# yglbgyx/DS-GAN

Hardware: AMD Instinct MI355X
Metric: 256×256 paired imgs/sec (G+D step) at 1/2/4/8 MI355X; MS-SSIM Δ vs ref (higher is better)
Workload: dtype bf16; 1 GPU; DS-GAN optimize_parameters, MixConvNeXtML G + PatchGAN D + VGG16 perceptual + SSIM/L1/TV; global_batch=16, per_gpu_batch=16, parallelism=dp1, hip_graphs=True

## Files before the change

ds-gan_amd/csrc/mlp.hip:

```cpp
#include "common.h"
#include "lds_dma.h"
#include <type_traits>

namespace dsg {

typedef f32x16_t mf32x16;
typedef __attribute__((ext_vector_type(4))) short ms16x4;
typedef __attribute__((address_space(3))) ms16x4 lds_ms16x4;
typedef __attribute__((ext_vector_type(4))) unsigned int mu32x4;

template <typename T16>
__device__ __forceinline__ hx8<T16> mtr_frag(const T16* p0, int stride) {
#if defined(__HIP_DEVICE_COMPILE__)
  ms16x4 lo = __builtin_amdgcn_ds_read_tr16_b64_v4i16((lds_ms16x4*)(p0));
  ms16x4 hi = __builtin_amdgcn_ds_read_tr16_b64_v4i16((lds_ms16x4*)(p0 + 4 * stride));
  typedef __attribute__((ext_vector_type(8))) short s16x8;
  s16x8 v = {lo[0], lo[1], lo[2], lo[3], hi[0], hi[1], hi[2], hi[3]};
  return __builtin_bit_cast(hx8<T16>, v);
#else
  return hx8<T16>{};
#endif
}

template <typename T16>
// ... 8 lines not shown
template <bool PK>
__device__ __forceinline__ void mlp_gelu_pair2(f32x2 z, f32x2& g, f32x2& gp) {
  if (PK) gelu_pair_fast2(z, g, gp);
  else gelu_pair_fast1x2(z, g, gp);
}
template <bool PK>
__device__ __forceinline__ f32x2 mlp_mul2(f32x2 a, f32x2 b) { return PK ? a * b : f32x2{a.x * b.x, a.y * b.y}; }

struct MlpArgs {
  const void* h; long h_bs;
  const float* dy; long dy_bs;
  const void* w1;
  const float* b1;
  const void* w2;
  const float* b2;
  float* out; long out_bs;
  void* g_out;
  void* dz_out;
  float* bsum;
  int HW, nb, accumulate;
  int h_bf16;
  float* ws;
  int splits;
  const float* x; long x_bs;
  const void* wsc;
};

__device__ __forceinline__ int xcd_tile(int id, int nwg) {
  const int xcd = id & 7, q = nwg >> 3, r = nwg & 7;
  return (xcd < r ? xcd * (q + 1) : r * (q + 1) + (xcd - r) * q) + (id >> 3);
}

template <int K, int BN, int STR, int NT, typename T16>
__device__ __forceinline__ void stage_rows(T16* dst, const float* __restrict__ src, int HW, int tid) {
  constexpr int ITEMS = K * BN / 4;
  static_assert(ITEMS % NT == 0, "tile must split evenly over the workgroup");
  constexpr int PER = ITEMS / NT;
  constexpr int BATCH = PER < 8 ? PER : 8;
#pragma unroll
  for (int i0 = 0; i0 < PER; i0 += BATCH) {
    float4 v[BATCH];
#pragma unroll
    for (int i = 0; i < BATCH; ++i) {
      const int it = tid + (i0 + i) * NT;
      const int k = it / (BN / 4), c4 = it % (BN / 4);
      v[i] = *reinterpret_cast<const float4*>(src + (long)k * HW + c4 * 4);
    }
// ... 450 lines not shown
  return __builtin_bit_cast(hx8<T16>, v);
#else
  return hx8<T16>{};
#endif
}
template <int S, typename T16>
__device__ __forceinline__ hx8<T16> mtr_frag_s(const T16* T, int k0, int col0, int lane) {
#if defined(__HIP_DEVICE_COMPILE__)
  const int tq = (lane >> 2) & 3, tp = lane & 3, tG = (lane >> 4) & 1, h = lane >> 5;
  const int col = col0 + 16 * tG + 4 * tp;
  const int rlo = k0 + 8 * h + tq, rhi = rlo + 4;
  const T16* plo = T + rlo * (S * 8) + (((col >> 3) ^ slot_swz<S>(rlo)) << 3) + (col & 7);
  const T16* phi = T + rhi * (S * 8) + (((col >> 3) ^ slot_swz<S>(rhi)) << 3) + (col & 7);
  ms16x4 lo = __builtin_amdgcn_ds_read_tr16_b64_v4i16((lds_ms16x4*)(plo));
  ms16x4 hi = __builtin_amdgcn_ds_read_tr16_b64_v4i16((lds_ms16x4*)(phi));
  typedef __attribute__((ext_vector_type(8))) short s16x8;
  s16x8 v = {lo[0], lo[1], lo[2], lo[3], hi[0], hi[1], hi[2], hi[3]};
  return __builtin_bit_cast(hx8<T16>, v);
#else
  return hx8<T16>{};
#endif
}

template <typename T16, int C, int P, int MINB>
__global__ __launch_bounds__(512, MINB) void mlp_dh_kernel(MlpArgs g) {
  typedef hx8<T16> mbf16x8;
  typedef hx4<T16> mbf16x4;
  constexpr int NW = 8, NT = NW * 64, BN = 128, HC = 64;
  constexpr int C4 = 4 * C, NCH = C4 / HC, KS = C / 16, PS = P / 16, CT = C / 32;
  constexpr int HSTR = BN + 32;
  constexpr int ST_SZ = (C + P) * HSTR, W_SZ = HC * C + P * HC, R_SZ = 2 * 4 * CT * 16 * 64;
  constexpr int SM = ST_SZ > 2 * W_SZ ? (ST_SZ > R_SZ ? ST_SZ : R_SZ) : (2 * W_SZ > R_SZ ? 2 * W_SZ : R_SZ);
  __shared__ __attribute__((aligned(16))) T16 smem[SM + 2 * C4];
  float* b1s = reinterpret_cast<float*>(smem + SM);
  static_assert(C % 64 == 0 && P % 64 == 0 && NCH >= 2, "tile shape");

  const int tid = threadIdx.x, lane = tid & 63, wave = __builtin_amdgcn_readfirstlane(tid >> 6);
  const int lr = lane & 31, lh = lane >> 5;
  const int tq = (lane >> 2) & 3, tp = lane & 3, tG = (lane >> 4) & 1;
  const int wm = wave >> 2, wn = wave & 3;

  const int tpi = g.HW / BN;
  const int tile = xcd_tile(blockIdx.x, gridDim.x);
  const int img = tile / tpi, p0 = (tile - img * tpi) * BN;

  T16* Hs = smem;
  T16* Ds = smem + C * HSTR;
// ... 64 lines not shown
    raw_barrier();
    if (j + 2 < NCH) {
      T16* W1n = smem + (j & 1) * W_SZ;
      glds_chunk<C, P, NW, false>(W1n, W1n + HC * C, g.w1, g.w2, j + 2, wave, lane);
    }
  }

  float* red = reinterpret_cast<float*>(smem);
#pragma unroll
  for (int ct = 0; ct < CT; ++ct)
    if ((ct & 1) != wm)
#pragma unroll
      for (int r = 0; r < 16; ++r) red[((wn * CT + ct) * 16 + r) * 64 + lane] = hacc[ct][r];
  __syncthreads();
  float* ob = g.out + (long)img * g.out_bs + p0 + wn * 32 + lr;
#pragma unroll
  for (int ct = 0; ct < CT; ++ct)
    if ((ct & 1) == wm)
#pragma unroll
      for (int r = 0; r < 16; ++r) {
        const float o = red[((wn * CT + ct) * 16 + r) * 64 + lane];
        ob[(long)(ct * 32 + (r & 3) + 8 * (r >> 2) + 4 * lh) * g.HW] = wm == 0 ? hacc[ct][r] + o : o + hacc[ct][r];
      }
}

template <typename T16, int C, int P, int BN, int HC, int NW, bool GD, int MINB, bool DMA = false>
__global__ __launch_bounds__(NW * 64, MINB) void mlp_bwd_kernel(MlpArgs g) {
  typedef hx8<T16> mbf16x8;
  typedef hx4<T16> mbf16x4;
  constexpr int NT = NW * 64;
  constexpr int C4 = 4 * C, NCH = C4 / HC;
  constexpr int HSTR = BN + 32, NSTR = HC, W1STR = C, W2STR = HC;
  constexpr int H_SZ = C * HSTR, D_SZ = P * HSTR, N_SZ = BN * NSTR, W1_SZ = HC * W1STR, W2_SZ = P * W2STR;
  constexpr int W_SZ = W1_SZ + W2_SZ;
  static_assert(!DMA || (H_SZ + D_SZ >= W_SZ && HC == 64 && (C / 8) % NW == 0 && (P / 8) % NW == 0), "DMA ring");
  constexpr int SM_SZ = DMA ? H_SZ + D_SZ + W_SZ + (GD ? 2 : 1) * N_SZ + 2 * C4
                            : H_SZ + D_SZ + (GD ? 2 : 1) * N_SZ + W1_SZ + W2_SZ;
  __shared__ __attribute__((aligned(16))) T16 smem[SM_SZ];
  T16* Hs = smem;
  T16* Ds = Hs + H_SZ;
  T16* Zn = Ds + D_SZ + (DMA ? W_SZ : 0);
  T16* Gn = Zn + (GD ? N_SZ : 0);
  T16* W1s = DMA ? Ds + D_SZ : Zn + (GD ? 2 : 1) * N_SZ;
  T16* W2s = W1s + W1_SZ;
  float* b1s = reinterpret_cast<float*>(Zn + (GD ? 2 : 1) * N_SZ);

  using ZG = WGrid<HC, BN, NW>;
  using HG = WGrid<C, BN, NW>;
  static_assert(P % 16 == 0 && HC == 64 && BN % 16 == 0, "tile shape");
// ... 142 lines not shown
          hacc[i][t] = mfma16(af[i], bf[t], hacc[i][t]);
    }
    if constexpr (!DMA) {
      __syncthreads();
      if (j + 1 < NCH) {
        wch_store_swz<C, P, HC, NT>(wr1, wr2, W1s, W2s, tid);
        __syncthreads();
      }
    }
  }

  float* ob = g.out + (long)img * g.out_bs + p0;
#pragma unroll
  for (int i = 0; i < HG::TM; ++i)
#pragma unroll
    for (int t = 0; t < HG::TN; ++t) {
      const int n = wn * (BN / HG::WN) + t * 32 + lr;
#pragma unroll
      for (int r = 0; r < 16; ++r) {
        const int c = wm * (C / 2) + i * 32 + (r & 3) + 8 * (r >> 2) + 4 * lh;
        ob[(long)c * g.HW + n] = hacc[i][t][r];
      }
    }
}

template <int S>
__device__ __forceinline__ unsigned swz_row_b(int row, int lh) {
  return (unsigned)(row * S * 16 + ((lh ^ slot_swz<S>(row)) << 4));
}
template <int S>
__device__ __forceinline__ uint2 swz_tr_b(int col0, int lane) {
  const int tq = (lane >> 2) & 3, tp = lane & 3, tG = (lane >> 4) & 1, h = lane >> 5;
  const int col = col0 + 16 * tG + 4 * tp;
  const int rlo = 8 * h + tq, rhi = rlo + 4;
  return make_uint2((unsigned)(rlo * S * 8 + (((col >> 3) ^ slot_swz<S>(rlo)) << 3) + (col & 7)) * 2u,
                    (unsigned)(rhi * S * 8 + (((col >> 3) ^ slot_swz<S>(rhi)) << 3) + (col & 7)) * 2u);
}
template <typename T16>
__device__ __forceinline__ hx8<T16> tr_at(const T16* T, uint2 a, unsigned k_bytes) {
#if defined(__HIP_DEVICE_COMPILE__)
  const char* b = (const char*)T + k_bytes;
  ms16x4 lo = __builtin_amdgcn_ds_read_tr16_b64_v4i16((lds_ms16x4*)(b + a.x));
  ms16x4 hi = __builtin_amdgcn_ds_read_tr16_b64_v4i16((lds_ms16x4*)(b + a.y));
  typedef __attribute__((ext_vector_type(8))) short s16x8;
  s16x8 v = {lo[0], lo[1], lo[2], lo[3], hi[0], hi[1], hi[2], hi[3]};
  return __builtin_bit_cast(hx8<T16>, v);
#else
  return hx8<T16>{};
#endif
}

template <typename T16, int C, int P>
__global__ __launch_bounds__(256, 1) void mlp_bwd_dma_kernel(MlpArgs g) {
  typedef hx8<T16> mbf16x8;
  typedef hx4<T16> mbf16x4;
  constexpr int NW = 4, NT = 256, BN = 64, HC = 64;
  constexpr int C4 = 4 * C, NCH = C4 / HC;
  constexpr int HSTR = BN + 32;
  constexpr int H_SZ = C * HSTR, D_SZ = P * HSTR, N_SZ = BN * HC, W1_SZ = HC * C, W2_SZ = P * HC;
  constexpr int W_SZ = W1_SZ + W2_SZ;
  static_assert(H_SZ + D_SZ >= W_SZ && NCH % 2 == 0 && (C / 8) % NW == 0 && (P / 8) % NW == 0, "shape");
  __shared__ __attribute__((aligned(1024))) T16 smem[H_SZ + D_SZ + W_SZ + 2 * N_SZ + 2 * C4];
  T16* const Hs = smem;
  T16* const Ds = Hs + H_SZ;
  T16* const Wslot0 = Ds + D_SZ;
  T16* const Wslot1 = Hs;
  T16* const Zn = Wslot0 + W_SZ;
  T16* const Gn = Zn + N_SZ;
  float* const b1s = reinterpret_cast<float*>(Gn + N_SZ);

  const int tid = threadIdx.x, lane = tid & 63, wave = __builtin_amdgcn_readfirstlane(tid >> 6);
  const int lr = lane & 31, lh = lane >> 5;
  const int tq = (lane >> 2) & 3, tp = lane & 3, tG = (lane >> 4) & 1;
  const int wm = wave >> 1, wn = wave & 1;

// ... 118 lines not shown
      dzb[ks] = *reinterpret_cast<const mbf16x8*>((const char*)Zn + (a_n ^ (unsigned)(32 * ks)));
#pragma unroll
      for (int i = 0; i < 4; ++i) w1t[ks][i] = tr_at(W1s, a_d[i], ks * 16 * C * 2);
    }
    __builtin_amdgcn_sched_barrier(0);
#pragma unroll
    for (int ks = 0; ks < HC / 16; ++ks)
#pragma unroll
      for (int i = 0; i < 4; ++i) hacc[i] = mfma16(w1t[ks][i], dzb[ks], hacc[i]);
  };
  for (int j = 0; j < NCH; j += 2) {
    chunk(j, Wslot0, Wslot1);
    chunk(j + 1, Wslot1, Wslot0);
  }

  float* ob = g.out + (long)img * g.out_bs + p0 + wn * 32 + lr;
#pragma unroll
  for (int i = 0; i < 4; ++i)
#pragma unroll
    for (int r = 0; r < 16; ++r) {
      const int c = wm * (C / 2) + i * 32 + (r & 3) + 8 * (r >> 2) + 4 * lh;
      ob[(long)c * g.HW] = hacc[i][r];
    }
}

template <int K, int BN, int NT, bool BF>
struct TileLd {
  static constexpr int E = BF ? 8 : 4;
  static constexpr int N = K * BN / E / NT;
  static_assert((K * BN / E) % NT == 0, "tile split");
  mu32x4 v[N];
  __device__ __forceinline__ void load(const void* src, int HW, int tid) {
#pragma unroll
    for (int i = 0; i < N; ++i) {
      const int it = tid + i * NT, k = it / (BN / E), c = it % (BN / E);
      const char* p = (const char*)src + ((long)k * HW + c * E) * (BF ? 2 : 4);
      v[i] = *reinterpret_cast<const mu32x4*>(p);
    }
  }
  template <int STR, typename T16>
  __device__ __forceinline__ void store(T16* dst, int tid) const {
#pragma unroll
    for (int i = 0; i < N; ++i) {
      const int it = tid + i * NT, k = it / (BN / E), c = it % (BN / E);
      if constexpr (BF) *reinterpret_cast<mu32x4*>(dst + k * STR + c * E) = v[i];
      else *reinterpret_cast<hx4<T16>*>(dst + k * STR + c * E) = mcvt4<T16>(__builtin_bit_cast(float4, v[i]));
// ... 268 lines not shown
static int mlp_bn(int C, int P) {
  if ((C == 64 && P == 128) || (C == 128 && P == 64) || (C == 128 && P == 256) || (C == 256 && P == 128)) return 128;
  return 0;
}
constexpr int MLP_NW = 8;

template <typename T16, int C, int P, int BN, int MINB>
static void fwd_lds_launch(const MlpArgs& g, hipStream_t st) {
  const unsigned tiles = (unsigned)((long)g.nb * (g.HW / BN));
  if (g.x)
    hipLaunchKernelGGL((mlp_fwd_lds_kernel<T16, C, P, BN, 64, MLP_NW, MINB, true>), dim3(tiles), dim3(MLP_NW * 64), 0, st,
                       g);
  else
    hipLaunchKernelGGL((mlp_fwd_lds_kernel<T16, C, P, BN, 64, MLP_NW, MINB>), dim3(tiles), dim3(MLP_NW * 64), 0, st, g);
}
template <typename T16, int C, int P, int MINB>
static void fwd_launch(const MlpArgs& g, hipStream_t st) {
  const unsigned tiles = (unsigned)((long)g.nb * (g.HW / 128));
  if (g.x) hipLaunchKernelGGL((mlp_fwd_kernel<T16, C, P, MINB, true>), dim3(tiles), dim3(512), 0, st, g);
  else hipLaunchKernelGGL((mlp_fwd_kernel<T16, C, P, MINB>), dim3(tiles), dim3(512), 0, st, g);
}
static int g_mlp_tune[4] = {2, 0, 0, 0};

template <typename T16, int C, int P, int BN, int NW, bool GD = true, int MINB = 1, bool DMA = false>
static void bwd_launch(const MlpArgs& g, hipStream_t st) {
  static_assert(BN / (NW / 2) == 32, "bsum granularity");
  const unsigned tiles = (unsigned)((long)g.nb * (g.HW / BN));
  hipLaunchKernelGGL((mlp_bwd_kernel<T16, C, P, BN, 64, NW, GD, MINB, DMA>), dim3(tiles), dim3(NW * 64), 0, st, g);
}

static int mlp_wgrad_splits(int C, int P, int HW, int nb) {
  const int bn = 64;
  const int nch = 4 * C / 64;
  const long ntiles = (long)nb * (HW / bn);
  long S = 512 / nch;
  S = S / 8 * 8;
  if (S < 8) S = 8;
  if (S > ntiles) S = ntiles;
  return (int)S;
}

template <typename T16, int C, int P, int BN, int NW, int MINB>
static void wgrad_launch(const MlpArgs& g, hipStream_t st) {
  const unsigned wgs = (unsigned)((4 * C / 64) * g.splits);
  if (g.h_bf16) hipLaunchKernelGGL((mlp_wgrad_kernel<T16, C, P, BN, NW, true, MINB>), dim3(wgs), dim3(NW * 64), 0, st, g);
  else hipLaunchKernelGGL((mlp_wgrad_kernel<T16, C, P, BN, NW, false, MINB>), dim3(wgs), dim3(NW * 64), 0, st, g);
}

}

using namespace dsg;
// ... 23 lines not shown
    using T16 = std::remove_pointer_t<decltype(t)>;
    if (C == 64) fwd_lds_launch<T16, 64, 128, 128, 2>(g, st);
    else if (C == 128 && P == 64) fwd_launch<T16, 128, 64, 4>(g, st);
    else if (C == 128) fwd_launch<T16, 128, 256, 2>(g, st);
    else fwd_launch<T16, 256, 128, 2>(g, st);
  });
  DSG_CHECK_LAUNCH();
  return 0;
}

int dsgan_mlp_fwd(const void* h, long h_bs, int h_bf16, const void* w1, const float* b1, const void* w2,
                  const float* b2, float* out, long out_bs, int nb, int C, int P, int HW,
                  int accumulate, hipStream_t st) {
  return mlp_fwd_impl(h, h_bs, h_bf16, w1, b1, w2, b2, nullptr, 0, nullptr, out, out_bs, nb, C, P, HW, accumulate, st);
}

int dsgan_mlp_fwd_sc(const void* h, long h_bs, int h_bf16, const void* w1, const float* b1, const void* w2,
                     const float* b2, const float* x, long x_bs, const void* ws, float* out, long out_bs, int nb,
                     int C, int P, int HW, int accumulate, hipStream_t st) {
  DSG_REQUIRE(x && ws, "dsgan_mlp_fwd_sc: bad args");
  return mlp_fwd_impl(h, h_bs, h_bf16, w1, b1, w2, b2, x, x_bs, ws, out, out_bs, nb, C, P, HW, accumulate, st);
}

int dsgan_mlp_bwd(const void* h, long h_bs, int h_bf16, const float* dy, long dy_bs, const void* w1, const float* b1,
                  const void* w2, float* dh, long dh_bs, void* g_out, void* dz_out, float* bsum, int nb,
                  int C, int P, int HW, hipStream_t st) {
  DSG_REQUIRE(h && dy && w1 && b1 && w2 && dh && nb > 0 && (g_out != nullptr) == (dz_out != nullptr) && (g_out || !bsum),
              "dsgan_mlp_bwd: bad args (g_out and dz_out both or neither; bsum needs them)");
  DSG_REQUIRE(dsgan_mlp_supported(C, P, HW), "dsgan_mlp_bwd: unsupported shape C=%d P=%d HW=%d", C, P, HW);
  DSG_REQUIRE(((uintptr_t)h & 15) == 0 && ((uintptr_t)dy & 15) == 0 && (h_bs & 7) == 0 && (dy_bs & 3) == 0 &&
              ((uintptr_t)g_out & 15) == 0 && ((uintptr_t)dz_out & 15) == 0,
              "dsgan_mlp_bwd: operands must be 16-byte aligned");
  MlpArgs g{};
  g.h = h; g.h_bs = h_bs; g.dy = dy; g.dy_bs = dy_bs; g.w1 = w1; g.b1 = b1;
  g.w2 = w2; g.out = dh; g.out_bs = dh_bs; g.g_out = g_out;
  g.dz_out = dz_out; g.bsum = bsum; g.HW = HW; g.nb = nb; g.h_bf16 = h_bf16;
  with_half([&](auto* t) {
    using T16 = std::remove_pointer_t<decltype(t)>;
    if (!g_out) {
      const unsigned tiles = (unsigned)((long)g.nb * (g.HW / 128));
      if (C == 64) hipLaunchKernelGGL((mlp_dh_kernel<T16, 64, 128, 2>), dim3(tiles), dim3(512), 0, st, g);
      else if (C == 128 && P == 64) hipLaunchKernelGGL((mlp_dh_kernel<T16, 128, 64, 2>), dim3(tiles), dim3(512), 0, st, g);
      else if (C == 128) bwd_launch<T16, 128, 256, 64, 4, false, 1>(g, st);
      else bwd_launch<T16, 256, 128, 64, 4, false, 1>(g, st);
    } else if (C == 64) bwd_launch<T16, 64, 128, 128, 8>(g, st);
    else if (C == 128 && P == 64) bwd_launch<T16, 128, 64, 128, 8>(g, st);
    else if (C == 128) bwd_launch<T16, 128, 256, 64, 4>(g, st);
    else if (g_mlp_tune[0] == 2 && P == 128)
      hipLaunchKernelGGL((mlp_bwd_dma_kernel<T16, 256, 128>), dim3((unsigned)((long)g.nb * (g.HW / 64))), dim3(256), 0,
                         st, g);
    else if (g_mlp_tune[0] == 0) bwd_launch<T16, 256, 128, 64, 4, true, 1, true>(g, st);
    else bwd_launch<T16, 256, 128, 64, 4>(g, st);
  });
  DSG_CHECK_LAUNCH();
  return 0;
}

long dsgan_mlp_wgrad_workspace(int C, int P, int HW, int nb) {
  if (!dsgan_mlp_supported(C, P, HW)) return 0;
  const long S = mlp_wgrad_splits(C, P, HW, nb);
  return S * (4L * C * C + (long)P * 4 * C + 4L * C);
}

int dsgan_mlp_wgrad(const void* h, long h_bs, int h_bf16, const float* dy, long dy_bs, const void* w1,
                    const float* b1, const void* w2, float* dw1, float* db1, float* dw2, float* ws, long ws_elems,
                    int nb, int C, int P, int HW, hipStream_t st) {
  DSG_REQUIRE(h && dy && w1 && b1 && w2 && dw1 && db1 && dw2 && nb > 0, "dsgan_mlp_wgrad: bad args");
  DSG_REQUIRE(dsgan_mlp_supported(C, P, HW), "dsgan_mlp_wgrad: unsupported shape C=%d P=%d HW=%d", C, P, HW);
  DSG_REQUIRE(((uintptr_t)h & 15) == 0 && ((uintptr_t)dy & 15) == 0 && (h_bs & 7) == 0 && (dy_bs & 3) == 0,
              "dsgan_mlp_wgrad: operands must be 16-byte aligned");
  MlpArgs g{};
  g.h = h; g.h_bs = h_bs; g.h_bf16 = h_bf16; g.dy = dy; g.dy_bs = dy_bs; g.w1 = w1; g.b1 = b1;
  g.w2 = w2; g.HW = HW; g.nb = nb; g.ws = ws;
  const int S = mlp_wgrad_splits(C, P, HW, nb);
  g.splits = S;
  DSG_WS((long)S * (4L * C * C + (long)P * 4 * C + 4L * C), ws, ws_elems, "dsgan_mlp_wgrad (dsgan_mlp_wgrad_workspace)");
  with_half([&](auto* t) {
    using T16 = std::remove_pointer_t<decltype(t)>;
// ... 44 lines not shown
```

ds-gan_amd/dsgan_hip/_lib.py:

```python
import ctypes
import os

import torch

_HERE = os.path.dirname(os.path.abspath(__file__))
LIB_PATH = os.environ.get("DSGAN_HIP_LIB", os.path.join(_HERE, "libdsgan_hip.so"))

P = ctypes.c_void_p
L = ctypes.c_long
I = ctypes.c_int
F = ctypes.c_float
D = ctypes.c_double
S = ctypes.c_void_p

SIGNATURES = {
    "dsgan_abi_version": [],
    "dsgan_set_half_type": [ctypes.c_int],
    "dsgan_amp_parts": [],
    "dsgan_amp_check": [P, L, P, P, F, F, I, S],
    "dsgan_adam_amp": [P, P, P, P, L, D, D, D, D, P, S],
    "dsgan_get_half_type": [],
    "dsgan_clear_launch_error": [],
    "dsgan_ktimer": [I],
    "dsgan_ktimer_read": [P, I],
# ... 2 lines not shown
    "dsgan_last_ws_need": [],
    "dsgan_conv_fwd": [P, L, P, P, P, L, P, L] + [I] * 12 + [F, I, I, I, S],
    "dsgan_conv_dgrad": [P, L, P, P, P, L, P, L, P, L, I, I, I, I, I, I, I, I, I, I, I, I, I, F, I, I, S],
    "dsgan_conv_wgrad": [P, L, P, L, P] + [I] * 13 + [P, L, S],
    "dsgan_conv_wgrad_workspace": [I] * 8,
    "dsgan_pw_supported": [I, I, I, I, L, L, P, P],
    "dsgan_pw_gemm": [I, P, L, P, L, P, L, P, P, L, P, L, I, I, I, I, I, I, I, I, I, F, P, L, S],
    "dsgan_pw_wgrad_workspace": [I, I, I, I],
    "dsgan_pw_wgrad_mixed": [P, L, I, P, L, I, P, P, I, I, I, I, P, L, S],
    "dsgan_pw_fwd_io": [P, I, P, L, I, P, L, I, P, L, I, P, I, I, I, I, I, I, F, S],
    "dsgan_pw_dgrad_io": [P, I, P, L, I, P, L, I, P, L, I, I, I, I, I, S],
    "dsgan_pw_fwd_io_ws": [P, I, P, L, I, P, L, I, P, L, I, P, I, I, I, I, I, I, F, P, L, S],
    "dsgan_pw_dgrad_io_ws": [P, I, P, L, I, P, L, I, P, L, I, I, I, I, I, P, L, S],
    "dsgan_pw_fd_workspace": [I, I, I, I, I],
    "dsgan_wtrans_multi": [P, P, P, I, S],
    "dsgan_pw_tune": [I, I],
    "dsgan_pw_f32_supported": [I, I, I, I, L, L, P, P],
    "dsgan_pw_f32_wgrad_workspace": [I, I, I, I],
    "dsgan_pw_gemm_f32": [I, P, L, P, L, P, L, P, P, L, I, I, I, I, I, I, I, I, F, P, L, S],
    "dsgan_mlp_supported": [I, I, I],
    "dsgan_mlp_fwd": [P, L, I, P, P, P, P, P, L, I, I, I, I, I, S],
    "dsgan_mlp_fwd_sc": [P, L, I, P, P, P, P, P, L, P, P, L, I, I, I, I, I, S],
    "dsgan_mlp_bwd": [P, L, I, P, L, P, P, P, P, L, P, P, P, I, I, I, I, S],
    "dsgan_mlp_wgrad_workspace": [I, I, I, I],
    "dsgan_mlp_wgrad": [P, L, I, P, L, P, P, P, P, P, P, P, L, I, I, I, I, S],
    "dsgan_mlp_tune": [I, I],
    "dsgan_colsum": [P, I, I, P, S],
    "dsgan_split_defer": [I],
    "dsgan_split_pending": [],
    "dsgan_split_flush": [S],
    "dsgan_f32_to_bf16": [P, P, L, S],
    "dsgan_pconv_supported": [I, I, I, I],
    "dsgan_conv_wtrans_bf16": [P, P, I, I, I, I, I, S],
    "dsgan_pconv": [P, L, P, P, P, L, P, L] + [I] * 13 + [F, I, S],
    "dsgan_pconv_workspace": [I] * 5,
    "dsgan_pconv_ws": [P, L, P, P, P, L, P, L] + [I] * 13 + [F, I, P, L, S],
    "dsgan_pw_small_supported": [I, I, I, L, L],
    "dsgan_pw_small": [P, L, P, I, I, P, P, L, P, L] + [I] * 8 + [F, S],
    "dsgan_pw_small2": [P, L, P, I, I, P, L, P, I, P, P, L, P, L] + [I] * 8 + [F, S],
    "dsgan_pconvt_supported": [I, I, I, I],
    "dsgan_pconvt": [P, L, P, P, P, L, P, L] + [I] * 11 + [F, I, S],
    "dsgan_pconvt_tune": [I, I],
    "dsgan_wconv_supported": [I, I, I, I],
    "dsgan_wconv_workspace": [I, I, I, I, I, I, I],
    "dsgan_wconv": [P, L, P, L, P, P, L] + [I] * 11 + [S],
    "dsgan_wconv_db": [P, L, P, L, P, P, P, L] + [I] * 11 + [S],
# ... 122 lines not shown


def load():
    global _lib
    if _lib is not None:
        return _lib
    if not os.path.exists(LIB_PATH):
        raise RuntimeError(
            "libdsgan_hip.so not found at %s -- build it with `python ds-gan_amd/build_lib.py` "
            "(there is no CPU/PyTorch fallback for the DS-GAN hot path)" % LIB_PATH)
    lib = ctypes.CDLL(LIB_PATH)
    for name, argtypes in SIGNATURES.items():
        fn = getattr(lib, name)
        fn.argtypes = argtypes
        fn.restype = (ctypes.c_char_p if name == "dsgan_last_error_string"
                      else ctypes.c_long if name.endswith(("_workspace", "_parts", "_size", "_need", "_plan")) else ctypes.c_int)
    _lib = lib
    return lib


DEFER_HOOK = [None]


def call(name, *args):
    lib = load()
    hook = DEFER_HOOK[0]
    n0 = lib.dsgan_split_pending() if hook is not None else 0
    rc = getattr(lib, name)(*args)
    if hook is not None:
        hook(lib.dsgan_split_pending() > n0)
    if rc != 0:
        msg = lib.dsgan_last_error_string()
        raise RuntimeError("%s failed (rc=%d): %s" % (name, rc, msg.decode() if msg else ""))


def ptr(t):
    if t is None:
        return None
    if not t.is_cuda:
        raise RuntimeError("dsgan_hip: expected a device tensor, got %s on %s" % (tuple(t.shape), t.device))
    return t.data_ptr()


def stream():
    return torch.cuda.current_stream().cuda_stream
```

ds-gan_amd/dsgan_hip/functional.py:

```python
import contextlib
import ctypes
import os
import math

import torch

from . import _lib
from ._lib import call, ptr, stream


def wsa(t):
    if t is not None and _DEFER_KEEP[0] is not None:
        _DEFER_CAND.append(t)
    return (ptr(t), t.numel() if t is not None else 0)


DEFER_SPLITS = [os.environ.get("DSGAN_DEFER_SPLITS", "1") != "0"]
_DEFER_KEEP = [None]
_DEFER_CAND = []


def _defer_hook(queued):
    if queued and _DEFER_KEEP[0] is not None:
        _DEFER_KEEP[0].extend(_DEFER_CAND)
# ... 150 lines not shown
        return out

    def table(self):
        torch.cuda.synchronize()
        return [(r[0].elapsed_time(r[1]), r[2], r[3] + (r[4],)) for r in self.rec]


IGEMM_TIMER = KernelTimer(kernel_only=True)
AUX_TIMER = KernelTimer()


class _timed:
    __slots__ = ("timer", "rec", "e0")

    def __init__(self, timer, flops, tag=None, fam="other", nbytes=0):
        self.timer, self.rec = timer, (flops, tag, fam, nbytes)

    def __enter__(self):
        self.e0 = self.timer.begin()

    def __exit__(self, etype, exc, tb):
        if etype is None:
            self.timer.end(self.e0, *self.rec)


def _ws(query, *dims, like):
    n = getattr(_lib.load(), query)(*dims)
    return torch.empty(n, device=like.device, dtype=torch.float32) if n > 0 else None


def _nb(*ts):
    return float(sum(t.numel() * t.element_size() for t in ts if t is not None))


def _conv_flops(N, Cin, Cout, KH, KW, Ho, Wo):
    return 2.0 * N * Cout * Cin * KH * KW * Ho * Wo


def _in_act(act):
    return ACT_GELU_FAST if act == "gelu" and _state["prec"] != "fp32" else ACT[act]


def nchw(t):
    if t.dim() != 4:
        raise ValueError("expected NCHW tensor, got %s" % (tuple(t.shape),))
    N, C, H, W = t.shape
# ... 744 lines not shown
        x, w, b = ctx.saved_tensors
        dx = conv_fwd_raw(dy, w, None, 2, 1) if ctx.needs_input_grad[0] else None
        gw = _grad_buf(ctx.w_ref) if ctx.needs_input_grad[1] else None
        if gw is not None:
            conv_wgrad_raw(x, dy, gw, 2, 1)
        gb = _grad_buf(ctx.b_ref) if (b is not None and ctx.needs_input_grad[2]) else None
        if gb is not None:
            channel_sum_raw(dy, gb)
        _params_done(ctx.w_ref, ctx.b_ref)
        return _give(ctx.box, dx), None, None


def conv_transpose3s2(x, w, b):
    return ConvT3s2Fn.apply(x, w, b)



def _mlp_tile(C, P, HW, x):
    if not _is16() or x.data_ptr() % 16:
        return 0
    return int(_lib.load().dsgan_mlp_supported(C, P, HW))


MLP_FOLD_SC = [os.environ.get("DSGAN_MLP_FOLD_SC", "1") != "0"]


def _mlp_flops(N, C, P, HW):
    return 2.0 * N * HW * (4 * C * C + 4 * C * P)


class PwMlpFn(torch.autograd.Function):

    @staticmethod
    def forward(ctx, h, x, w1, b1, w2, b2, ws, norm=False, slot=None, acc=None):
        N, C, H, W = h.shape
        P, HW, C4 = w2.shape[0], H * W, 4 * C
        if acc is not None:
            if (slot is not None or tuple(acc.shape) != (N, P, H, W) or acc.dtype != torch.float32
                    or not acc.is_contiguous()):
                raise ValueError("pw_mlp: acc must be a dense fp32 [%d,%d,%d,%d] tensor (no slot)" % (N, P, H, W))
            ctx.mark_dirty(acc)
        ctx.box_acc = _box(acc) if acc is not None else None
        out0 = slot.tail() if slot is not None else acc
        acc1 = acc is not None
        obs = nchw(out0)[1] if out0 is not None else P * HW
        ctx.refs = (w1, b1, w2, b2, ws)
        ctx.prec = _state["prec"]
# ... 101 lines not shown
            conv_wgrad_raw(dy, x, gws, 1, 0)

    @staticmethod
    def _gdz_wgrads(ctx, dy, dybs, g, dz, h, x, grads):
        gw2, gb2, gws, gw1, gb1 = grads
        N, C, H, W = h.shape
        HW, C4, P = H * W, 4 * C, dy.shape[1]
        if gw2 is not None:
            with _timed(IGEMM_TIMER, 2.0 * N * HW * C4 * P, ("wgrad", N, C4, H, W, P, 1, 1), "pwgemm_kernel",
                        _nb(dy, g, gw2)):
                call("dsgan_pw_wgrad_mixed", ptr(dy), dybs, 0, ptr(g), C4 * HW, 1, ptr(gw2), ptr(gb2), P, C4, HW, N,
                     *wsa(_pw_ws(P, C4, HW, N, dy)), stream())
            gb2 = None
        PwMlpFn._b2_sc(dy, x, gb2, gws)
        if gw1 is not None:
            with _timed(IGEMM_TIMER, 2.0 * N * HW * C4 * C, ("wgrad", N, C, H, W, C4, 1, 1), "pwgemm_kernel",
                        _nb(dz, h, gw1)):
                call("dsgan_pw_wgrad_mixed", ptr(dz), C4 * HW, 1, ptr(h), C * HW, ctx.hb, ptr(gw1), ptr(gb1), C4, C,
                     HW, N, *wsa(_pw_ws(C4, C, HW, N, dz)), stream())
        elif gb1 is not None:
            channel_sum_raw(dz.float(), gb1)

    @staticmethod
    def _done(ctx, dy, ws, x):
        _params_done(*ctx.refs)
        if not ctx.needs_input_grad[1]:
            return None
        out, acc = _acc_target(ctx.box_x)
        dx = conv_dgrad_raw(dy, ws, tuple(x.shape), 1, 0, out=out, accumulate=acc)
        return None if acc else _give(ctx.box_x, dx)

    @staticmethod
    def _backward_unfused(ctx, dy):
        h, x, z, w1v, w2v, ws = ctx.saved_tensors
        w1, b1, w2, b2, ws_ref = ctx.refs
        dy, dybs = nchw(dy)
        if dy.data_ptr() % 16 or dybs % 8:
            dy = dy.contiguous()
            dybs = dy.shape[1] * dy.shape[2] * dy.shape[3]
        grads = gw2, gb2, gws, gw1, gb1 = tuple(_grad_buf(t) for t in (w2, b2, ws_ref, w1, b1))
        want_dh = ctx.needs_input_grad[0]
        if ctx.g is not None:
            N, C4, H, W = z.shape
            HW, P, C = H * W, w2.shape[0], h.shape[1]
            dz = torch.empty((N, C4, H, W), device=dy.device, dtype=half_dtype())
            with _timed(IGEMM_TIMER, 2.0 * N * HW * C4 * P, ("dgrad", N, C4, H, W, P, 1, 1), "pwgemm_kernel",
                        _nb(dy, w2, dz, z)):
                call("dsgan_pw_dgrad_io_ws", ptr(bf16_weight(w2)), 1, ptr(dy), dybs, 0, ptr(dz), C4 * HW, 1, ptr(z),
                     C4 * HW, C4, P, HW, N, 0, *wsa(_ws("dsgan_pw_fd_workspace", 1, C4, P, HW, N, like=dy)), stream())
            PwMlpFn._gdz_wgrads(ctx, dy, dybs, ctx.g, dz, h, x, grads)
            dh = None
            if want_dh:
                dh = _empty(N, C, H, W, dy)
                with _timed(IGEMM_TIMER, 2.0 * N * HW * C4 * C, ("dgrad", N, C4, H, W, C, 1, 1), "pwgemm_kernel",
                            _nb(dz, w1, dh)):
                    call("dsgan_pw_dgrad_io_ws", ptr(bf16_weight(w1)), 1, ptr(dz), C4 * HW, 1, ptr(dh), C * HW, 0, None,
                         0, C, C4, HW, N, 0, *wsa(_ws("dsgan_pw_fd_workspace", 1, C, C4, HW, N, like=dz)), stream())
            return dh, PwMlpFn._done(ctx, dy, ws, x)
        dz = conv_dgrad_raw(dy, w2v, tuple(z.shape), 1, 0, gpre=z, gact="gelu")
        if gw2 is not None and conv_wgrad_raw(dy, z, gw2.view(w2v.shape), 1, 0, xact="gelu", db=gb2):
            gb2 = None
        PwMlpFn._b2_sc(dy, x, gb2, gws)
        if gw1 is not None and conv_wgrad_raw(dz, h, gw1.view(w1v.shape), 1, 0, db=gb1):
            gb1 = None
        if gb1 is not None:
            channel_sum_raw(dz, gb1)
        dh = conv_dgrad_raw(dz, w1v, tuple(h.shape), 1, 0) if want_dh else None
        return dh, PwMlpFn._done(ctx, dy, ws, x)

    @staticmethod
    def _backward_fused(ctx, dy):
        h, x, ws = ctx.saved_tensors
        w1, b1, w2, b2, ws_ref = ctx.refs
        N, C, H, W = h.shape
        HW, C4, P = H * W, 4 * h.shape[1], w2.shape[0]
        dy, dybs = nchw(dy)
        if dy.data_ptr() % 16:
            dy, dybs = dy.contiguous(), P * HW
        grads = gw2, gb2, gws, gw1, gb1 = tuple(_grad_buf(t) for t in (w2, b2, ws_ref, w1, b1))
        dh = _empty(N, C, H, W, h)
        if gw1 is not None and gb1 is not None and gw2 is not None and C < 256:
            w1b, w2b = bf16_weight(w1), bf16_weight(w2)
            with _timed(IGEMM_TIMER, 2.0 * N * HW * C4 * (2 * C + P), ("mlp_bwd", N, C, H, W, P, 1, 1),
                        "mlp_bwd_kernel", _nb(h, dy, w1, b1, w2, dh)):
                call("dsgan_mlp_bwd", ptr(h), C * HW, ctx.hb, ptr(dy), dybs, ptr(w1b), ptr(b1), ptr(w2b), ptr(dh),
                     C * HW, None, None, None, N, C, P, HW, stream())
            with _timed(IGEMM_TIMER, 2.0 * N * HW * C4 * (2 * C + 2 * P), ("mlp_wgrad", N, C, H, W, P, 1, 1),
                        "mlp_wgrad_kernel", _nb(h, dy, w1, b1, w2, gw1, gb1, gw2)):
                call("dsgan_mlp_wgrad", ptr(h), C * HW, ctx.hb, ptr(dy), dybs, ptr(w1b), ptr(b1), ptr(w2b), ptr(gw1),
                     ptr(gb1), ptr(gw2), *wsa(_ws("dsgan_mlp_wgrad_workspace", C, P, HW, N, like=h)), N, C, P, HW,
                     stream())
            PwMlpFn._b2_sc(dy, x, gb2, gws)
            return dh, PwMlpFn._done(ctx, dy, ws, x)
        g = torch.empty((N, C4, H, W), device=h.device, dtype=half_dtype())
        dz = torch.empty_like(g)
        with _timed(IGEMM_TIMER, _mlp_flops(N, C, P, HW), ("mlp_bwd", N, C, H, W, P, 1, 1), "mlp_bwd_kernel",
                    _nb(h, dy, w1, b1, w2, dh, g, dz)):
            call("dsgan_mlp_bwd", ptr(h), C * HW, ctx.hb, ptr(dy), dybs, ptr(bf16_weight(w1)), ptr(b1),
                 ptr(bf16_weight(w2)), ptr(dh), C * HW, ptr(g), ptr(dz), None, N, C, P, HW, stream())
        PwMlpFn._gdz_wgrads(ctx, dy, dybs, g, dz, h, x, grads)
        return dh, PwMlpFn._done(ctx, dy, ws, x)


def pw_mlp(h, x, w1, b1, w2, b2, ws, norm=False, slot=None, acc=None):
    return PwMlpFn.apply(h, x, w1, b1, w2, b2, ws, norm, slot, acc)



def dwconv_raw(x, w, b, flip=False, out=None, accumulate=False):
    x, xbs = nchw(x)
    N, C, H, W = x.shape
    K = w.shape[-1]
    y = out if out is not None else _empty(N, C, H, W, x)
    y4, ybs = nchw(y)
    with _timed(AUX_TIMER, 2.0 * N * C * H * W * K * K, ("dw_dgrad" if flip else "dw_fwd", N, C, H, W, K), "dwconv",
                (3 if accumulate else 2) * _nb(x)):
        call("dsgan_dwconv_fwd", ptr(x), xbs, ptr(w), ptr(b), ptr(y4), ybs, N, C, H, W, K, int(flip), int(accumulate),
             stream())
    return y4


def _dw_wgrad(dy, x, gw, gb, K):
    dy4, dybs = nchw(dy)
    x4, xbs = nchw(x)
# ... 1333 lines not shown
```

include/dsgan_hip.h:

```cpp
#ifndef DSGAN_HIP_H
#define DSGAN_HIP_H

#include <hip/hip_runtime.h>

#ifdef __cplusplus
extern "C" {
#endif

int dsgan_abi_version(void);
const char* dsgan_last_error_string(void);
int dsgan_set_plan_only(int on);
long dsgan_last_ws_need(void);
int dsgan_set_half_type(int t);
int dsgan_get_half_type(void);
int dsgan_clear_launch_error(void);
int dsgan_ktimer(int on);
int dsgan_ktimer_read(float* ms, int max);

int dsgan_conv_fwd(const float* x, long x_bs, const float* w, const float* bias, float* y,
                   long y_bs, float* ypre, long ypre_bs, int N, int Cin, int H, int W, int Cout,
                   int KH, int KW, int stride, int pad, int Ho, int Wo, int act, float slope,
                   int accumulate, int xact, int prec, hipStream_t stream);
int dsgan_conv_dgrad(const float* dy, long dy_bs, const float* w, const float* bias, float* dx,
                     long dx_bs, float* ypre, long ypre_bs, const float* gpre, long gpre_bs,
// ... 27 lines not shown
int dsgan_pw_fwd_io(const void* W, int w_bf16, const void* X, long x_bs, int x_bf16, void* Y, long y_bs, int y_bf16,
                    const void* ypre, long ypre_bs, int ypre_grad_bf16, const float* bias, int M, int K, int P, int nb,
                    int act, int accumulate, float slope, hipStream_t stream);
int dsgan_pw_fwd_io_ws(const void* W, int w_bf16, const void* X, long x_bs, int x_bf16, void* Y, long y_bs, int y_bf16,
                       const void* ypre, long ypre_bs, int ypre_grad_bf16, const float* bias, int M, int K, int P,
                       int nb, int act, int accumulate, float slope, float* ws, long ws_elems, hipStream_t stream);
int dsgan_pw_dgrad_io(const void* W, int w_bf16, const void* DY, long dy_bs, int dy_bf16, void* DX, long dx_bs,
                      int dx_bf16, const void* GP, long gp_bs, int M, int K, int P, int nb, int accumulate,
                      hipStream_t stream);
int dsgan_pw_dgrad_io_ws(const void* W, int w_bf16, const void* DY, long dy_bs, int dy_bf16, void* DX, long dx_bs,
                         int dx_bf16, const void* GP, long gp_bs, int M, int K, int P, int nb, int accumulate,
                         float* ws, long ws_elems, hipStream_t stream);

int dsgan_mlp_supported(int C, int P, int HW);
int dsgan_mlp_fwd(const void* h, long h_bs, int h_bf16, const void* w1, const float* b1, const void* w2,
                  const float* b2, float* out, long out_bs, int nb, int C, int P, int HW,
                  int accumulate, hipStream_t stream);
int dsgan_mlp_fwd_sc(const void* h, long h_bs, int h_bf16, const void* w1, const float* b1, const void* w2,
                     const float* b2, const float* x, long x_bs, const void* ws, float* out, long out_bs, int nb,
                     int C, int P, int HW, int accumulate, hipStream_t stream);
int dsgan_mlp_bwd(const void* h, long h_bs, int h_bf16, const float* dy, long dy_bs, const void* w1,
                  const float* b1, const void* w2, float* dh, long dh_bs, void* g_out, void* dz_out,
                  float* bsum, int nb, int C, int P, int HW, hipStream_t stream);
long dsgan_mlp_wgrad_workspace(int C, int P, int HW, int nb);
int dsgan_mlp_wgrad(const void* h, long h_bs, int h_bf16, const float* dy, long dy_bs, const void* w1,
                    const float* b1, const void* w2, float* dw1, float* db1, float* dw2, float* ws, long ws_elems,
                    int nb, int C, int P, int HW, hipStream_t stream);
int dsgan_mlp_tune(int key, int val);
int dsgan_colsum(float* part, int rows, int cols, float* out, hipStream_t stream);

int dsgan_split_defer(int on);
int dsgan_split_pending(void);
int dsgan_split_flush(hipStream_t stream);
int dsgan_f32_to_bf16(const float* src, void* dst, long n, hipStream_t stream);

int dsgan_conv_small_out(const float* x, long x_bs, const float* w, long wm, long wk, long wh, long ww,
                         const float* bias, float* y, long y_bs, int nb, int K, int M, int Hin, int Win,
                         int Ho, int Wo, int KH, int KW, int stride, int pad, int transposed,
                         int accumulate, hipStream_t stream);
int dsgan_conv_small_in(const float* x, long x_bs, const float* w, long wm, long wk, long wh, long ww,
                        const float* bias, float* y, long y_bs, int nb, int K, int M, int Hin, int Win,
                        int Ho, int Wo, int KH, int KW, int stride, int pad, int transposed, int act,
                        float slope, int accumulate, hipStream_t stream);
long dsgan_conv_wgrad_small_workspace(int N, int Cin, int Cout, int KH, int KW, int Ho, int Wo);
int dsgan_conv_wgrad_small(const float* dy, long dy_bs, const float* x, long x_bs, float* dw, int N,
                           int Cin, int H, int W, int Cout, int KH, int KW, int stride, int pad, int Ho,
// ... 293 lines not shown
```

Before: 681.5 img/s.

## Fold shortcut 1x1 dgrad into MLP backward kernels epilogue

Adds an SC variant of the MLP backward kernels (dh, bwd, dma) that, after writing dh, stages the shortcut weight Ws into LDS and computes the shortcut input gradient dx from the dy fragments already held in registers, writing or accumulating into dx. Python backward calls the new dsgan_mlp_bwd_sc entry when shapes and alignment allow, falling back to the separate conv_dgrad otherwise. This removes a separate dgrad launch and a second read of dy, at the cost of extra LDS staging, register pressure and longer kernel tails.

```diff
diff --git a/ds-gan_amd/csrc/mlp.hip b/ds-gan_amd/csrc/mlp.hip
--- a/ds-gan_amd/csrc/mlp.hip
+++ b/ds-gan_amd/csrc/mlp.hip
@@ -54,7 +54,8 @@
   int h_bf16;
   float* ws;
   int splits;
-  const float* x; long x_bs;
+  union { const float* x; float* dx; };
+  union { long x_bs; long dx_bs; };
   const void* wsc;
 };
 
@@ -551,7 +552,49 @@
 #endif
 }
 
-template <typename T16, int C, int P, int MINB>
+template <typename T16, int C, int P, int NT>
+__device__ __forceinline__ void sc_stage_ws(T16* Wt, const void* wsc, int tid) {
+  constexpr int STR = C + 32, ITEMS = P * C / 8;
+  static_assert(ITEMS % NT == 0, "Ws must split evenly over the workgroup");
+  constexpr int PER = ITEMS / NT, BATCH = PER < 8 ? PER : 8;
+  const mu32x4* __restrict__ src = reinterpret_cast<const mu32x4*>(wsc);
+#pragma unroll
+  for (int i0 = 0; i0 < PER; i0 += BATCH) {
+    mu32x4 v[BATCH];
+#pragma unroll
+    for (int i = 0; i < BATCH; ++i) v[i] = src[tid + (i0 + i) * NT];
+#pragma unroll
+    for (int i = 0; i < BATCH; ++i) {
+      const int it = tid + (i0 + i) * NT, row = it / (C / 8), c8 = it % (C / 8);
+      *reinterpret_cast<mu32x4*>(Wt + row * STR + c8 * 8) = v[i];
+    }
+  }
+}
+template <typename T16, int C, int P>
+__device__ __forceinline__ void sc_dx_tile(const T16* Wt, const hx8<T16> (&db)[P / 16], int c0, float* d0, int HW,
+                                           int accumulate, int lane) {
+  constexpr int STR = C + 32;
+  const int lh = lane >> 5, tq = (lane >> 2) & 3, tp = lane & 3, tG = (lane >> 4) & 1;
+  const T16* a0 = Wt + (8 * lh + tq) * STR + c0 + 16 * tG + 4 * tp;
+  mf32x16 s;
+#pragma unroll
+  for (int r = 0; r < 16; ++r) s[r] = 0.f;
+#pragma unroll
+  for (int ks = 0; ks < P / 16; ++ks) s = mfma16(mtr_frag(a0 + ks * 16 * STR, STR), db[ks], s);
+  float* d = d0 + (long)(c0 + 4 * lh) * HW;
+  if (accumulate) {
+    float o[16];
+#pragma unroll
+    for (int r = 0; r < 16; ++r) o[r] = d[(long)((r & 3) + 8 * (r >> 2)) * HW];
+#pragma unroll
+    for (int r = 0; r < 16; ++r) d[(long)((r & 3) + 8 * (r >> 2)) * HW] = o[r] + s[r];
+  } else {
+#pragma unroll
+    for (int r = 0; r < 16; ++r) d[(long)((r & 3) + 8 * (r >> 2)) * HW] = s[r];
+  }
+}
+
+template <typename T16, int C, int P, int MINB, bool SC = false>
 __global__ __launch_bounds__(512, MINB) void mlp_dh_kernel(MlpArgs g) {
   typedef hx8<T16> mbf16x8;
   typedef hx4<T16> mbf16x4;
@@ -662,9 +705,20 @@
         const float o = red[((wn * CT + ct) * 16 + r) * 64 + lane];
         ob[(long)(ct * 32 + (r & 3) + 8 * (r >> 2) + 4 * lh) * g.HW] = wm == 0 ? hacc[ct][r] + o : o + hacc[ct][r];
       }
-}
-
-template <typename T16, int C, int P, int BN, int HC, int NW, bool GD, int MINB, bool DMA = false>
+  if constexpr (SC) {
+    static_assert(P * (C + 32) <= SM, "Ws tile");
+    __syncthreads();
+    const int ln = (int)__builtin_amdgcn_mbcnt_hi(~0u, __builtin_amdgcn_mbcnt_lo(~0u, 0u));
+    sc_stage_ws<T16, C, P, NT>(smem, g.wsc, wave * 64 + ln);
+    __syncthreads();
+    float* xb = g.dx + (long)img * g.dx_bs + p0 + wn * 32 + (ln & 31);
+#pragma unroll
+    for (int ct = 0; ct < CT; ++ct)
+      if ((ct & 1) == wm) sc_dx_tile<T16, C, P>(smem, db, ct * 32, xb, g.HW, g.accumulate, ln);
+  }
+}
+
+template <typename T16, int C, int P, int BN, int HC, int NW, bool GD, int MINB, bool DMA = false, bool SC = false>
 __global__ __launch_bounds__(NW * 64, MINB) void mlp_bwd_kernel(MlpArgs g) {
   typedef hx8<T16> mbf16x8;
   typedef hx4<T16> mbf16x4;
@@ -853,6 +907,16 @@
         ob[(long)c * g.HW + n] = hacc[i][t][r];
       }
     }
+  if constexpr (SC) {
+    static_assert(HG::TN == 1 && P * (C + 32) <= SM_SZ, "Ws tile");
+    __syncthreads();
+    sc_stage_ws<T16, C, P, NT>(smem, g.wsc, tid);
+    __syncthreads();
+    float* xb = g.dx + (long)img * g.dx_bs + p0 + wn * (BN / HG::WN) + lr;
+#pragma unroll
+    for (int i = 0; i < HG::TM; ++i)
+      sc_dx_tile<T16, C, P>(smem, dbr, wm * (C / 2) + i * 32, xb, g.HW, g.accumulate, lane);
+  }
 }
 
 template <int S>
@@ -881,7 +945,7 @@
 #endif
 }
 
-template <typename T16, int C, int P>
+template <typename T16, int C, int P, bool SC = false>
 __global__ __launch_bounds__(256, 1) void mlp_bwd_dma_kernel(MlpArgs g) {
   typedef hx8<T16> mbf16x8;
   typedef hx4<T16> mbf16x4;
@@ -1046,6 +1110,16 @@
       const int c = wm * (C / 2) + i * 32 + (r & 3) + 8 * (r >> 2) + 4 * lh;
       ob[(long)c * g.HW] = hacc[i][r];
     }
+  if constexpr (SC) {
+    static_assert(P * (C + 32) <= H_SZ + D_SZ + W_SZ, "Ws tile");
+    __syncthreads();
+    const int ln = (int)__builtin_amdgcn_mbcnt_hi(~0u, __builtin_amdgcn_mbcnt_lo(~0u, 0u));
+    sc_stage_ws<T16, C, P, NT>(smem, g.wsc, wave * 64 + ln);
+    __syncthreads();
+    float* xb = g.dx + (long)img * g.dx_bs + p0 + wn * 32 + (ln & 31);
+#pragma unroll
+    for (int i = 0; i < 4; ++i) sc_dx_tile<T16, C, P>(smem, dbr, wm * (C / 2) + i * 32, xb, g.HW, g.accumulate, ln);
+  }
 }
 
 template <int K, int BN, int NT, bool BF>
@@ -1360,11 +1434,27 @@
 }
 static int g_mlp_tune[4] = {2, 0, 0, 0};
 
+constexpr int MLP_NO_SC_FORM = -2;
+static bool mlp_bwd_sc_form(int C, int P, bool gd) { return mlp_bn(C, P) != 0 && (!gd || C == 256); }
+
 template <typename T16, int C, int P, int BN, int NW, bool GD = true, int MINB = 1, bool DMA = false>
 static void bwd_launch(const MlpArgs& g, hipStream_t st) {
   static_assert(BN / (NW / 2) == 32, "bsum granularity");
   const unsigned tiles = (unsigned)((long)g.nb * (g.HW / BN));
+  if constexpr (!GD || C == 256) {
+    if (g.dx) {
+      hipLaunchKernelGGL((mlp_bwd_kernel<T16, C, P, BN, 64, NW, GD, MINB, DMA, true>), dim3(tiles), dim3(NW * 64), 0, st,
+                         g);
+      return;
+    }
+  }
   hipLaunchKernelGGL((mlp_bwd_kernel<T16, C, P, BN, 64, NW, GD, MINB, DMA>), dim3(tiles), dim3(NW * 64), 0, st, g);
+}
+template <typename T16, int C, int P>
+static void dh_launch(const MlpArgs& g, hipStream_t st) {
+  const unsigned tiles = (unsigned)((long)g.nb * (g.HW / 128));
+  if (g.dx) hipLaunchKernelGGL((mlp_dh_kernel<T16, C, P, 2, true>), dim3(tiles), dim3(512), 0, st, g);
+  else hipLaunchKernelGGL((mlp_dh_kernel<T16, C, P, 2>), dim3(tiles), dim3(512), 0, st, g);
 }
 
 static int mlp_wgrad_splits(int C, int P, int HW, int nb) {
@@ -1434,9 +1524,12 @@
   return mlp_fwd_impl(h, h_bs, h_bf16, w1, b1, w2, b2, x, x_bs, ws, out, out_bs, nb, C, P, HW, accumulate, st);
 }
 
-int dsgan_mlp_bwd(const void* h, long h_bs, int h_bf16, const float* dy, long dy_bs, const void* w1, const float* b1,
-                  const void* w2, float* dh, long dh_bs, void* g_out, void* dz_out, float* bsum, int nb,
-                  int C, int P, int HW, hipStream_t st) {
+long dsgan_pw_fd_workspace(int mode, int M, int K, int P, int nb);
+
+static int mlp_bwd_impl(const void* h, long h_bs, int h_bf16, const float* dy, long dy_bs, const void* w1,
+                        const float* b1, const void* w2, float* dh, long dh_bs, void* g_out, void* dz_out, float* bsum,
+                        const void* ws, float* dx, long dx_bs, int accumulate, int nb, int C, int P, int HW,
+                        hipStream_t st) {
   DSG_REQUIRE(h && dy && w1 && b1 && w2 && dh && nb > 0 && (g_out != nullptr) == (dz_out != nullptr) && (g_out || !bsum),
               "dsgan_mlp_bwd: bad args (g_out and dz_out both or neither; bsum needs them)");
   DSG_REQUIRE(dsgan_mlp_supported(C, P, HW), "dsgan_mlp_bwd: unsupported shape C=%d P=%d HW=%d", C, P, HW);
@@ -1447,17 +1540,20 @@
   g.h = h; g.h_bs = h_bs; g.dy = dy; g.dy_bs = dy_bs; g.w1 = w1; g.b1 = b1;
   g.w2 = w2; g.out = dh; g.out_bs = dh_bs; g.g_out = g_out;
   g.dz_out = dz_out; g.bsum = bsum; g.HW = HW; g.nb = nb; g.h_bf16 = h_bf16;
+  g.wsc = ws; g.dx = dx; g.dx_bs = dx_bs; g.accumulate = accumulate;
   with_half([&](auto* t) {
     using T16 = std::remove_pointer_t<decltype(t)>;
     if (!g_out) {
-      const unsigned tiles = (unsigned)((long)g.nb * (g.HW / 128));
-      if (C == 64) hipLaunchKernelGGL((mlp_dh_kernel<T16, 64, 128, 2>), dim3(tiles), dim3(512), 0, st, g);
-      else if (C == 128 && P == 64) hipLaunchKernelGGL((mlp_dh_kernel<T16, 128, 64, 2>), dim3(tiles), dim3(512), 0, st, g);
+      if (C == 64) dh_launch<T16, 64, 128>(g, st);
+      else if (C == 128 && P == 64) dh_launch<T16, 128, 64>(g, st);
       else if (C == 128) bwd_launch<T16, 128, 256, 64, 4, false, 1>(g, st);
       else bwd_launch<T16, 256, 128, 64, 4, false, 1>(g, st);
     } else if (C == 64) bwd_launch<T16, 64, 128, 128, 8>(g, st);
     else if (C == 128 && P == 64) bwd_launch<T16, 128, 64, 128, 8>(g, st);
     else if (C == 128) bwd_launch<T16, 128, 256, 64, 4>(g, st);
+    else if (g_mlp_tune[0] == 2 && P == 128 && dx)
+      hipLaunchKernelGGL((mlp_bwd_dma_kernel<T16, 256, 128, true>), dim3((unsigned)((long)g.nb * (g.HW / 64))), dim3(256),
+                         0, st, g);
     else if (g_mlp_tune[0] == 2 && P == 128)
       hipLaunchKernelGGL((mlp_bwd_dma_kernel<T16, 256, 128>), dim3((unsigned)((long)g.nb * (g.HW / 64))), dim3(256), 0,
                          st, g);
@@ -1466,6 +1562,25 @@
   });
   DSG_CHECK_LAUNCH();
   return 0;
+}
+
+int dsgan_mlp_bwd(const void* h, long h_bs, int h_bf16, const float* dy, long dy_bs, const void* w1, const float* b1,
+                  const void* w2, float* dh, long dh_bs, void* g_out, void* dz_out, float* bsum, int nb,
+                  int C, int P, int HW, hipStream_t st) {
+  return mlp_bwd_impl(h, h_bs, h_bf16, dy, dy_bs, w1, b1, w2, dh, dh_bs, g_out, dz_out, bsum, nullptr, nullptr, 0, 0,
+                      nb, C, P, HW, st);
+}
+
+int dsgan_mlp_bwd_sc(const void* h, long h_bs, int h_bf16, const float* dy, long dy_bs, const void* w1,
+                     const float* b1, const void* w2, float* dh, long dh_bs, void* g_out, void* dz_out, float* bsum,
+                     const void* ws, float* dx, long dx_bs, int accumulate, int nb, int C, int P, int HW,
+                     hipStream_t st) {
+  DSG_REQUIRE(ws && dx && ((uintptr_t)ws & 15) == 0 && ((uintptr_t)dx & 15) == 0 && (dx_bs & 3) == 0,
+              "dsgan_mlp_bwd_sc: ws and dx must be 16-byte aligned, the dx batch stride a multiple of 4");
+  if (!mlp_bwd_sc_form(C, P, g_out != nullptr)) return MLP_NO_SC_FORM;
+  if (dsgan_pw_fd_workspace(1, C, P, HW, nb) != 0) return MLP_NO_SC_FORM;
+  return mlp_bwd_impl(h, h_bs, h_bf16, dy, dy_bs, w1, b1, w2, dh, dh_bs, g_out, dz_out, bsum, ws, dx, dx_bs,
+                      accumulate != 0, nb, C, P, HW, st);
 }
 
 long dsgan_mlp_wgrad_workspace(int C, int P, int HW, int nb) {
diff --git a/ds-gan_amd/dsgan_hip/_lib.py b/ds-gan_amd/dsgan_hip/_lib.py
--- a/ds-gan_amd/dsgan_hip/_lib.py
+++ b/ds-gan_amd/dsgan_hip/_lib.py
@@ -48,6 +48,7 @@
     "dsgan_mlp_fwd": [P, L, I, P, P, P, P, P, L, I, I, I, I, I, S],
     "dsgan_mlp_fwd_sc": [P, L, I, P, P, P, P, P, L, P, P, L, I, I, I, I, I, S],
     "dsgan_mlp_bwd": [P, L, I, P, L, P, P, P, P, L, P, P, P, I, I, I, I, S],
+    "dsgan_mlp_bwd_sc": [P, L, I, P, L, P, P, P, P, L, P, P, P, P, P, L, I, I, I, I, I, S],
     "dsgan_mlp_wgrad_workspace": [I, I, I, I],
     "dsgan_mlp_wgrad": [P, L, I, P, L, P, P, P, P, P, P, P, L, I, I, I, I, S],
     "dsgan_mlp_tune": [I, I],
@@ -216,6 +217,9 @@
 DEFER_HOOK = [None]
 
 
+DECLINED = {"dsgan_mlp_bwd_sc": -2}
+
+
 def call(name, *args):
     lib = load()
     hook = DEFER_HOOK[0]
@@ -224,8 +228,11 @@
     if hook is not None:
         hook(lib.dsgan_split_pending() > n0)
     if rc != 0:
+        if DECLINED.get(name) == rc:
+            return False
         msg = lib.dsgan_last_error_string()
         raise RuntimeError("%s failed (rc=%d): %s" % (name, rc, msg.decode() if msg else ""))
+    return True
 
 
 def ptr(t):
diff --git a/ds-gan_amd/dsgan_hip/functional.py b/ds-gan_amd/dsgan_hip/functional.py
--- a/ds-gan_amd/dsgan_hip/functional.py
+++ b/ds-gan_amd/dsgan_hip/functional.py
@@ -196,6 +196,9 @@
     def __exit__(self, etype, exc, tb):
         if etype is None:
             self.timer.end(self.e0, *self.rec)
+
+    def cancel(self):
+        self.e0 = None
 
 
 def _ws(query, *dims, like):
@@ -986,7 +989,12 @@
     return int(_lib.load().dsgan_mlp_supported(C, P, HW))
 
 
-MLP_FOLD_SC = [os.environ.get("DSGAN_MLP_FOLD_SC", "1") != "0"]
+def _env_switch(name):
+    return os.environ.get(name, "1") != "0"
+
+
+MLP_FOLD_SC = [_env_switch("DSGAN_MLP_FOLD_SC")]
+MLP_FOLD_SC_BWD = [_env_switch("DSGAN_MLP_FOLD_SC_BWD")]
 
 
 def _mlp_flops(N, C, P, HW):
@@ -1134,10 +1142,13 @@
             channel_sum_raw(dz.float(), gb1)
 
     @staticmethod
-    def _done(ctx, dy, ws, x):
+    def _done(ctx, dy, ws, x, folded=None):
         _params_done(*ctx.refs)
         if not ctx.needs_input_grad[1]:
             return None
+        if folded is not None:
+            dx, acc = folded
+            return None if acc else _give(ctx.box_x, dx)
         out, acc = _acc_target(ctx.box_x)
         dx = conv_dgrad_raw(dy, ws, tuple(x.shape), 1, 0, out=out, accumulate=acc)
         return None if acc else _give(ctx.box_x, dx)
@@ -1181,6 +1192,29 @@
         return dh, PwMlpFn._done(ctx, dy, ws, x)
 
     @staticmethod
+    def _data_path(ctx, flops, h, dy, dybs, dh, g, dz, ws, x):
+        w1, b1, w2 = ctx.refs[:3]
+        N, C, H, W = h.shape
+        HW, P = H * W, w2.shape[0]
+        tag, nbytes = ("mlp_bwd", N, C, H, W, P, 1, 1), _nb(h, dy, w1, b1, w2, dh, g, dz)
+        args = (ptr(h), C * HW, ctx.hb, ptr(dy), dybs, ptr(bf16_weight(w1)), ptr(b1), ptr(bf16_weight(w2)), ptr(dh),
+                C * HW, ptr(g), ptr(dz), None)
+        if MLP_FOLD_SC_BWD[0] and ctx.needs_input_grad[1] and ws.is_contiguous():
+            out, acc = _acc_target(ctx.box_x)
+            dx, dxbs = nchw(out if out is not None else _empty(*x.shape, x))
+            if dx.data_ptr() % 16 == 0 and dxbs % 4 == 0:
+                t = _timed(IGEMM_TIMER, flops + 2.0 * N * HW * C * P, tag, "mlp_bwd_kernel",
+                           nbytes + _nb(ws) + (2 if acc else 1) * _nb(dx))
+                with t:
+                    if call("dsgan_mlp_bwd_sc", *args, ptr(bf16_weight(ws)), ptr(dx), dxbs, int(acc), N, C, P, HW,
+                            stream()) is not False:
+                        return dx, acc
+                    t.cancel()
+        with _timed(IGEMM_TIMER, flops, tag, "mlp_bwd_kernel", nbytes):
+            call("dsgan_mlp_bwd", *args, N, C, P, HW, stream())
+        return None
+
+    @staticmethod
     def _backward_fused(ctx, dy):
         h, x, ws = ctx.saved_tensors
         w1, b1, w2, b2, ws_ref = ctx.refs
@@ -1193,25 +1227,19 @@
         dh = _empty(N, C, H, W, h)
         if gw1 is not None and gb1 is not None and gw2 is not None and C < 256:
             w1b, w2b = bf16_weight(w1), bf16_weight(w2)
-            with _timed(IGEMM_TIMER, 2.0 * N * HW * C4 * (2 * C + P), ("mlp_bwd", N, C, H, W, P, 1, 1),
-                        "mlp_bwd_kernel", _nb(h, dy, w1, b1, w2, dh)):
-                call("dsgan_mlp_bwd", ptr(h), C * HW, ctx.hb, ptr(dy), dybs, ptr(w1b), ptr(b1), ptr(w2b), ptr(dh),
-                     C * HW, None, None, None, N, C, P, HW, stream())
+            folded = PwMlpFn._data_path(ctx, 2.0 * N * HW * C4 * (2 * C + P), h, dy, dybs, dh, None, None, ws, x)
             with _timed(IGEMM_TIMER, 2.0 * N * HW * C4 * (2 * C + 2 * P), ("mlp_wgrad", N, C, H, W, P, 1, 1),
                         "mlp_wgrad_kernel", _nb(h, dy, w1, b1, w2, gw1, gb1, gw2)):
                 call("dsgan_mlp_wgrad", ptr(h), C * HW, ctx.hb, ptr(dy), dybs, ptr(w1b), ptr(b1), ptr(w2b), ptr(gw1),
                      ptr(gb1), ptr(gw2), *wsa(_ws("dsgan_mlp_wgrad_workspace", C, P, HW, N, like=h)), N, C, P, HW,
                      stream())
             PwMlpFn._b2_sc(dy, x, gb2, gws)
-            return dh, PwMlpFn._done(ctx, dy, ws, x)
+            return dh, PwMlpFn._done(ctx, dy, ws, x, folded)
         g = torch.empty((N, C4, H, W), device=h.device, dtype=half_dtype())
         dz = torch.empty_like(g)
-        with _timed(IGEMM_TIMER, _mlp_flops(N, C, P, HW), ("mlp_bwd", N, C, H, W, P, 1, 1), "mlp_bwd_kernel",
-                    _nb(h, dy, w1, b1, w2, dh, g, dz)):
-            call("dsgan_mlp_bwd", ptr(h), C * HW, ctx.hb, ptr(dy), dybs, ptr(bf16_weight(w1)), ptr(b1),
-                 ptr(bf16_weight(w2)), ptr(dh), C * HW, ptr(g), ptr(dz), None, N, C, P, HW, stream())
+        folded = PwMlpFn._data_path(ctx, _mlp_flops(N, C, P, HW), h, dy, dybs, dh, g, dz, ws, x)
         PwMlpFn._gdz_wgrads(ctx, dy, dybs, g, dz, h, x, grads)
-        return dh, PwMlpFn._done(ctx, dy, ws, x)
+        return dh, PwMlpFn._done(ctx, dy, ws, x, folded)
 
 
 def pw_mlp(h, x, w1, b1, w2, b2, ws, norm=False, slot=None, acc=None):
diff --git a/include/dsgan_hip.h b/include/dsgan_hip.h
--- a/include/dsgan_hip.h
+++ b/include/dsgan_hip.h
@@ -73,6 +73,10 @@
 int dsgan_mlp_bwd(const void* h, long h_bs, int h_bf16, const float* dy, long dy_bs, const void* w1,
                   const float* b1, const void* w2, float* dh, long dh_bs, void* g_out, void* dz_out,
                   float* bsum, int nb, int C, int P, int HW, hipStream_t stream);
+int dsgan_mlp_bwd_sc(const void* h, long h_bs, int h_bf16, const float* dy, long dy_bs, const void* w1,
+                     const float* b1, const void* w2, float* dh, long dh_bs, void* g_out, void* dz_out,
+                     float* bsum, const void* ws, float* dx, long dx_bs, int accumulate, int nb, int C, int P,
+                     int HW, hipStream_t stream);
 long dsgan_mlp_wgrad_workspace(int C, int P, int HW, int nb);
 int dsgan_mlp_wgrad(const void* h, long h_bs, int h_bf16, const float* dy, long dy_bs, const void* w1,
                     const float* b1, const void* w2, float* dw1, float* db1, float* dw2, float* ws, long ws_elems,
```

New measurement: 687.1 img/s, median of 6. No clear change (+0.8%).
